# dblalock/sprintz

Hardware: AMD Instinct MI355X
Metric: decompress MB/s (and ratio) uint16 rowmajor 8-col, 1/2/4/8 MI355X vs CPU ref (higher is better)
Workload: dtype u16

## Files before the change

sprintz_amd/csrc/decode_fast.h:

```cpp
#pragma once

#include "decode_kernel.h"
#include "group_ops.h"

namespace sprintz {

typedef uint32_t __attribute__((aligned(1), may_alias)) u32_unaligned;
typedef uint16_t __attribute__((aligned(1), may_alias)) u16_unaligned;
struct __attribute__((aligned(1), packed)) u128_unaligned { uint32_t x, y, z, w; };

typedef __attribute__((address_space(3))) const uint32_t lds_u32;
typedef __attribute__((address_space(3))) const uint8_t lds_u8;

__device__ __forceinline__ uint32_t lds_rd32(uint32_t a)
{
    lds_u32* q = (lds_u32*)(uintptr_t)(a & ~3u);
    return __builtin_amdgcn_alignbyte(q[1], q[0], a);
}
__device__ __forceinline__ uint32_t lds_rd8(uint32_t a) { return *(lds_u8*)(uintptr_t)a; }
__device__ __forceinline__ uint32_t lds_addr(const void* p)
{
    return (uint32_t)(uintptr_t)(__attribute__((address_space(3))) const void*)p;
}

__device__ __forceinline__ uint64_t wave_uniform64(uint64_t x)
{
    return ((uint64_t)(uint32_t)__builtin_amdgcn_readfirstlane((int)(uint32_t)(x >> 32)) << 32) |
           (uint64_t)(uint32_t)__builtin_amdgcn_readfirstlane((int)(uint32_t)x);
}

__device__ __forceinline__ int mad24(int a, int b, int c)
{
    int d;
    asm("v_mad_i32_i24 %0, %1, %2, %3" : "=v"(d) : "v"(a), "v"(b), "v"(c));
    return d;
}
__device__ __forceinline__ int sign_of(int x)
{
    int s;
    asm("v_med3_i32 %0, %1, -1, 1" : "=v"(s) : "v"(x));
    return s;
}

__device__ __forceinline__ int mad_i16_hi(int a, int b, int c)
{
    int d;
    asm("v_mad_i32_i16 %0, %1, %2, %3 op_sel:[1,0,0,0]" : "=v"(d) : "v"(a), "v"(b), "v"(c));
    return d;
}
__device__ __forceinline__ uint32_t add_hi16(uint32_t a, int x)
{
    uint32_t d;
    asm("v_add_u32_sdwa %0, %1, %2 dst_sel:DWORD dst_unused:UNUSED_PAD src0_sel:DWORD src1_sel:WORD_1" : "=v"(d) : "v"(a), "v"(x));
    return d;
}

template <int W, bool FIRE, int DP, int CPL, bool EXACT, int Q = 0, bool CM = false, int DS = 0>
__global__ void __launch_bounds__(kThreads) decode_fast_kernel(DecodeArgs a)
{
    using U = typename Elem<W>::U;
    typedef __attribute__((__vector_size__(4 * sizeof(uint32_t)))) uint32_t v4u;
    constexpr int HB = Elem<W>::HB;
    constexpr int ESZ = W / 8;
    constexpr int LOG2DP = DP == 4 ? 2 : DP == 8 ? 3 : DP == 16 ? 4 : DP == 32 ? 5 : 6;
    constexpr int DCAP = DP * CPL;
    constexpr uint32_t ROW16 = DP * 16;
    constexpr uint32_t UNIT = ROW16 * CPL;
    constexpr bool SPLIT = CPL == 3;
    static_assert(!SPLIT || (W == 8 && DP == 32 && !EXACT && !CM && Q == 0), "the split mapping is built for 8-bit row-major decodes");
    constexpr bool GATHER = Q == kQueryGather;
    static_assert(!GATHER || (!CM && !SPLIT && DS == 0), "gather: row-major destination, plain mappings");
    constexpr int DSZ = DS ? DS : DCAP;
    static_assert(DSZ <= DCAP, "sizing columns");
    constexpr uint32_t HDRMAX = (2 * DSZ * HB + 7) / 8;
    constexpr uint32_t BLKMAX = 8 * DSZ * ESZ;
    constexpr int PIECES = (BLKMAX + ROW16 - 1) / ROW16;
    constexpr uint32_t CG = HDRMAX + 2 * BLKMAX + 4;
    constexpr uint32_t NPEND = (CG + UNIT - 1) / UNIT;
    constexpr uint32_t CSTART = 16 + 8;
    constexpr uint32_t RBU = (2 * (CG + CSTART) + 3 + UNIT - 1) / UNIT + 1;
    constexpr uint32_t RB = RBU * UNIT;
    constexpr uint32_t APRON = (CG + CSTART + 8 + 15) & ~15u;
    static_assert(RB - UNIT >= 2 * (CG + CSTART) + 3, "ring too small for one step of read-ahead");
    static_assert(NPEND <= 3, "pending registers");
    extern __shared__ __attribute__((aligned(16))) uint8_t smem[];

    const int D = EXACT ? DCAP : a.D;
    const uint64_t gtid = (uint64_t)blockIdx.x * kThreads + threadIdx.x;
    const int lane_d = (int)(threadIdx.x & (uint32_t)(DP - 1));
    GatherPiece gp{};
    uint64_t c_sel = (gtid >> LOG2DP) * (uint64_t)a.chunks_per_group;
    if constexpr (GATHER) {
        if (!gather_piece(a, gtid >> LOG2DP, gp)) return;
        if (gp.exists && a.offsets[gp.chunk + 1] > 0xfffffff0ull - 4096u) { if (lane_d == 0) gather_fail(a, gp.range, kErrCorrupt); return; }
        if (!gp.exists) { if (lane_d == 0) gather_fail(a, gp.range, kErrNoRow); return; }
        c_sel = gp.chunk;
    }
    const uint64_t c_first = c_sel;
    if (c_first >= a.nchunks) return;
    const uint64_t c_end = GATHER ? c_first + 1 : (c_first + a.chunks_per_group < a.nchunks) ? c_first + a.chunks_per_group : a.nchunks;

    uint8_t* const ringp = smem + (size_t)(threadIdx.x >> LOG2DP) * a.lds_group_stride;
    const uint32_t ring = lds_addr(ringp);
    uint8_t* const stage = ringp + RB + APRON;

    const uint64_t wave_first = GATHER ? 0 : (((uint64_t)blockIdx.x * kThreads + (threadIdx.x & ~63u)) >> LOG2DP) * (uint64_t)a.chunks_per_group;
    uint64_t wave_base = 0;
    if constexpr (!GATHER) {
        wave_base = a.offsets[wave_first < a.nchunks ? wave_first : 0] & ~(uint64_t)15;
        wave_base = wave_uniform64(wave_base);
    }
    const uint64_t wave_span = ((a.offsets[a.nchunks] - wave_base) + 15) & ~(uint64_t)15;
    const __amdgpu_buffer_rsrc_t rsrc = __builtin_amdgcn_make_buffer_rsrc(
        (void*)(a.comp + wave_base), 0, (uint32_t)(wave_span < 0xffffffffull ? wave_span : 0xffffffffull), 0x00020000);
    const uint32_t rows_per_chunk = CM ? a.chunk_len / (uint32_t)(EXACT ? DCAP : a.D) : 0u;
    const uint64_t out_base = CM ? (wave_first < a.nchunks ? wave_first : 0) * (uint64_t)rows_per_chunk * ESZ
                                 : (wave_first < a.nchunks ? wave_first : 0) * (uint64_t)a.chunk_len * ESZ;
    const uint64_t out_span = CM ? (uint64_t)(EXACT ? DCAP : a.D) * a.col_stride * ESZ - out_base
                            : GATHER ? a.g_nranges * (uint64_t)a.g_rows * (uint64_t)(EXACT ? DCAP : a.D) * ESZ
                                 : a.nchunks * (uint64_t)a.chunk_len * ESZ - out_base;
    const __amdgpu_buffer_rsrc_t orsrc = __builtin_amdgcn_make_buffer_rsrc(
        (void*)((uint8_t*)a.out + wave_uniform64(out_base)), 0,
        (uint32_t)__builtin_amdgcn_readfirstlane((int)(uint32_t)(out_span < 0xfffffff0ull ? out_span : 0xfffffff0ull)), 0x00020000);
    constexpr uint32_t kDropStore = 0xfffffff0u;
#ifndef SPRINTZ_STORE_AUX
#define SPRINTZ_STORE_AUX 2
#endif
#ifndef SPRINTZ_DF_MERGE8
#define SPRINTZ_DF_MERGE8 1
#endif
    constexpr int kStoreAux = SPRINTZ_STORE_AUX;
    const uint32_t lane16 = (uint32_t)lane_d * 16u;
    uint64_t gabs = 0;
    uint32_t gvo = 0;
    uint32_t rp = 0;
    uint32_t rofs = 0;
    uint32_t ahead = 0;
    uint32_t cofs = lane16;

    uint4 pend[3][CPL];
    uint32_t npend = 0;

    auto request = [&](uint4 (&v)[CPL], bool wanted) {
#pragma unroll
        for (int j = 0; j < CPL; j++) {
            const auto t = __builtin_amdgcn_raw_buffer_load_b128(rsrc, wanted ? gvo + j * ROW16 : 0xfffffff0u, 0, 0);
            v[j] = make_uint4(t[0], t[1], t[2], t[3]);
        }
        gvo += wanted ? UNIT : 0u;
    };
    auto commit = [&](const uint4 (&v)[CPL]) {
#pragma unroll
        for (int j = 0; j < CPL; j++) {
            const uint32_t ro = cofs + j * ROW16;
            *(uint4*)(ringp + ro) = v[j];
            if (ro < APRON) *(uint4*)(ringp + RB + ro) = v[j];
        }
        cofs += UNIT;
        if (cofs >= RB) cofs -= RB;
    };
    auto prime = [&](uint64_t off) {
        gabs = off & ~(uint64_t)15;
        gvo = (uint32_t)(gabs - wave_base) + lane16;
        rp = (uint32_t)(off & 15);
        rofs = rp;
        cofs = lane16;
        npend = 0;
        wave_lds_sync();
#pragma unroll
        for (uint32_t u = 0; u < RB / UNIT; u++) {
            uint4 v[CPL];
            request(v, true);
            commit(v);
        }
        ahead = RB - rp;
        wave_lds_sync();
    };

    const uint32_t hdr_bytes = (2u * (uint32_t)D * HB + 7u) >> 3;
    const uint32_t blk_elems = 8u * (uint32_t)D;
    const uint32_t blk_bytes = blk_elems * ESZ;
    const uint32_t row_stride = (uint32_t)D * ESZ;
    const int col0 = lane_d * CPL;
    constexpr bool MERGE8 = SPRINTZ_DF_MERGE8 && W == 8 && (CPL % 2 == 0 || SPLIT) && !CM && Q == 0;
    const bool merge8 = MERGE8 && (EXACT || (D & 1) == 0);
    constexpr int NPAIR = CPL / 2;
    int genk[CPL];
    int colk[CPL];
    uint8_t* stage_k[CPL];
#pragma unroll
    for (int k = 0; k < CPL; k++) {
        genk[k] = SPLIT ? (k < 2 ? 2 * lane_d + k : 2 * DP + lane_d) : col0 + k;
        if (MERGE8 && merge8 && !SPLIT) {
            const int pb = (col0 + (k & ~1)) < D ? col0 + (k & ~1) : ((D - 1) & ~1);
            colk[k] = EXACT ? col0 + k : (pb + (k & 1) < D ? pb + (k & 1) : D - 1);
        } else {
            colk[k] = EXACT ? genk[k] : (genk[k] < D ? genk[k] : D - 1);
        }
        stage_k[k] = stage + colk[k] * ESZ;
    }

    uint32_t pv[CPL];
    int pd[CPL], ctr[CPL];
    bool col_ok[CPL];
#pragma unroll
    for (int k = 0; k < CPL; k++) { pv[k] = 0; pd[k] = 0; ctr[k] = 0; col_ok[k] = EXACT ? true : genk[k] < D; }
    uint32_t out_left = 0;
    bool corrupt = false;
    uint32_t qmax[CPL];
    uint64_t qsum[CPL];
    uint32_t qbs[CPL];
#pragma unroll
    for (int k = 0; k < CPL; k++) { qmax[k] = 0; qsum[k] = 0; qbs[k] = 0; }
    constexpr uint32_t MASK = Elem<W>::MASK;
    uint32_t qmin[CPL];
    uint32_t wi = 0, wleft = 0;
    uint64_t wbase = 0;
    auto q_row = [&](int k) {
        if constexpr (Q != 0) {
            if constexpr (W == 16) {
                asm("v_max_u32_sdwa %0, %1, %2 dst_sel:DWORD dst_unused:UNUSED_PAD src0_sel:DWORD src1_sel:WORD_0"
                    : "=v"(qmax[k]) : "v"(qmax[k]), "v"(pv[k]));
                if constexpr (Q == kQueryWindow)
                    asm("v_min_u32_sdwa %0, %1, %2 dst_sel:DWORD dst_unused:UNUSED_PAD src0_sel:DWORD src1_sel:WORD_0"
                        : "=v"(qmin[k]) : "v"(qmin[k]), "v"(pv[k]));
                asm("v_add_u32_sdwa %0, %1, %2 dst_sel:DWORD dst_unused:UNUSED_PAD src0_sel:DWORD src1_sel:WORD_0"
                    : "=v"(qbs[k]) : "v"(qbs[k]), "v"(pv[k]));
            } else {
                asm("v_max_u32_sdwa %0, %1, %2 dst_sel:DWORD dst_unused:UNUSED_PAD src0_sel:DWORD src1_sel:BYTE_0"
                    : "=v"(qmax[k]) : "v"(qmax[k]), "v"(pv[k]));
                if constexpr (Q == kQueryWindow)
                    asm("v_min_u32_sdwa %0, %1, %2 dst_sel:DWORD dst_unused:UNUSED_PAD src0_sel:DWORD src1_sel:BYTE_0"
                        : "=v"(qmin[k]) : "v"(qmin[k]), "v"(pv[k]));
                asm("v_add_u32_sdwa %0, %1, %2 dst_sel:DWORD dst_unused:UNUSED_PAD src0_sel:DWORD src1_sel:BYTE_0"
                    : "=v"(qbs[k]) : "v"(qbs[k]), "v"(pv[k]));
            }
        }
    };
    auto q_block = [&](int k) {
        if constexpr (Q != 0) { qsum[k] += qbs[k]; qbs[k] = 0; }
    };
    auto win_flush_all = [&]() {
#pragma unroll
        for (int k = 0; k < CPL; k++)
            if (col_ok[k]) win_flush<W>(a, (wbase + wi) * (uint64_t)D + (uint64_t)genk[k], qmin[k], qmax[k], qsum[k]);
        wi++;
        wleft = a.window_rows;
    };
    auto q_window = [&]() {
        if constexpr (Q == kQueryWindow) {
            wleft -= 8;
            if (wleft == 0) win_flush_all();
        }
    };
    uint32_t ovo = 0;
    uint32_t grow = 0;
    uint32_t prow[PIECES];
#pragma unroll
    for (int q = 0; q < PIECES; q++) prow[q] = GATHER ? (lane16 + (uint32_t)q * ROW16) / row_stride : 0u;
    const uint32_t gspan = gp.hi - gp.lo;

    uint4 held[2][PIECES];
    uint32_t held_vo[2][PIECES];
#pragma unroll
    for (int s2 = 0; s2 < 2; s2++)
#pragma unroll
        for (int q = 0; q < PIECES; q++) { held[s2][q] = make_uint4(0, 0, 0, 0); held_vo[s2][q] = kDropStore; }
    uint32_t pk[CPL][4];
    uint4 cheld[2][CPL];
    uint32_t cheld_vo[2][CPL];
    uint32_t cbase[CPL];
#pragma unroll
    for (int k = 0; k < CPL; k++) {
        cbase[k] = CM ? (uint32_t)((uint64_t)genk[k] * a.col_stride * ESZ) : 0u;
#pragma unroll
        for (int s2 = 0; s2 < 2; s2++) { cheld[s2][k] = make_uint4(0, 0, 0, 0); cheld_vo[s2][k] = kDropStore; }
    }
    auto store_col = [&](const uint4& t, uint32_t vo) {
        if constexpr (W == 16) {
            __builtin_amdgcn_raw_buffer_store_b128(__builtin_bit_cast(v4u, t), orsrc, vo, 0, kStoreAux);
        } else {
            typedef __attribute__((__vector_size__(2 * sizeof(uint32_t)))) uint32_t v2u;
            v2u h = {t.x, t.y};
            __builtin_amdgcn_raw_buffer_store_b64(h, orsrc, vo, 0, kStoreAux);
        }
    };
    constexpr bool CMB = CM && CPL == 1;
    constexpr uint32_t PB = W == 16 ? 16u : 8u;
    uint8_t* const cst = stage;
    uint32_t* const cvo = (uint32_t*)(stage + 4u * DCAP * PB);
    uint32_t stepno = 0;
    const uint32_t cs_bytes = CM ? (uint32_t)(a.col_stride * ESZ) : 0u;
    auto cst_at = [&](uint32_t col, uint32_t blk) { return cst + (col * 4u + ((blk + (col >> 2)) & 3u)) * PB; };
    if constexpr (CMB) {
        if (lane_d < 4) cvo[lane_d] = kDropStore;
        wave_lds_sync();
    }
    auto cm_flush = [&](bool real) {
        if constexpr (CMB) {
            wave_lds_sync();
#pragma unroll
            for (int j = 0; j < 4; j++) {
                const uint32_t pid = (uint32_t)j * DP + (uint32_t)lane_d, col = pid >> 2, p = pid & 3u;
                uint4 t = make_uint4(0, 0, 0, 0);
                uint32_t vo = kDropStore;
                if (real && col < (uint32_t)D) {
                    const uint32_t rofs_b = cvo[p];
                    if constexpr (W == 16) t = *(const uint4*)cst_at(col, p);
                    else { const uint2 h = *(const uint2*)cst_at(col, p); t.x = h.x; t.y = h.y; }
                    vo = rofs_b == kDropStore ? kDropStore : col * cs_bytes + rofs_b;
                }
                store_col(t, vo);
            }
            if (real) {
                wave_lds_sync();
                if (lane_d < 4) cvo[lane_d] = kDropStore;
            }
            wave_lds_sync();
        }
    };
    auto pack_row = [&](int k, int i) {
        if constexpr (CM) {
            if constexpr (W == 16) {
                if ((i & 1) == 0) pk[k][i >> 1] = pv[k] & 0xffffu;
                else pk[k][i >> 1] |= pv[k] << 16;
            } else {
                if ((i & 3) == 0) pk[k][i >> 2] = pv[k] & 0xffu;
                else pk[k][i >> 2] |= (pv[k] & 0xffu) << (8 * (i & 3));
            }
        }
    };
    auto stage_out = [&](int slot) {
        if constexpr (query_reduce_only(Q)) return;
        if constexpr (CMB) {
            if (slot >= 0) {
                const uint32_t blk = (stepno & 1u) * 2u + (uint32_t)slot;
                if (col_ok[0]) {
                    if constexpr (W == 16) *(uint4*)cst_at((uint32_t)col0, blk) = make_uint4(pk[0][0], pk[0][1], pk[0][2], pk[0][3]);
                    else *(uint2*)cst_at((uint32_t)col0, blk) = make_uint2(pk[0][0], pk[0][1]);
                }
                if (lane_d == 0) cvo[blk] = ovo;
            } else {
                const uint4 t = W == 16 ? make_uint4(pk[0][0], pk[0][1], pk[0][2], pk[0][3]) : make_uint4(pk[0][0], pk[0][1], 0, 0);
                store_col(t, col_ok[0] ? cbase[0] + ovo : kDropStore);
            }
            ovo += 8u * ESZ;
            return;
        }
        if constexpr (CM) {
#pragma unroll
            for (int k = 0; k < CPL; k++) {
                const uint4 t = W == 16 ? make_uint4(pk[k][0], pk[k][1], pk[k][2], pk[k][3]) : make_uint4(pk[k][0], pk[k][1], 0, 0);
                const uint32_t vo = col_ok[k] ? cbase[k] + ovo : kDropStore;
                if (slot >= 0) { cheld[slot][k] = t; cheld_vo[slot][k] = vo; }
                else store_col(t, vo);
            }
            ovo += 8u * ESZ;
            return;
        }
        wave_lds_sync();
#pragma unroll
        for (int q = 0; q < PIECES; q++) {
            const uint32_t u = lane16 + q * ROW16;
            bool in = u < blk_bytes;
            if constexpr (GATHER) in = in && grow + prow[q] - gp.lo < gspan;
            const uint4 t = *(const uint4*)(stage + (in ? u : 0u));
            if (slot >= 0) {
                held[slot][q] = t;
#ifdef SPRINTZ_ABL_NO_GSTORE
                held_vo[slot][q] = kDropStore;
#elif defined(SPRINTZ_ABL_STORE_INTERLEAVE)
                {
                    const uint32_t g = (threadIdx.x & 63u) >> LOG2DP, gbase = g * a.chunk_len * ESZ;
                    held_vo[slot][q] = in ? ((ovo - gbase) >> 7) * 1024u + g * 128u + u : kDropStore;
                }
#elif defined(SPRINTZ_ABL_STORE_SLOT0_ONLY)
                held_vo[slot][q] = (in && slot == 0) ? ovo + u : kDropStore;
#elif defined(SPRINTZ_ABL_STORE_HALF_LANES)
                held_vo[slot][q] = (in && (lane_d & 1) == 0) ? ovo + u : kDropStore;
#else
                held_vo[slot][q] = in ? ovo + u : kDropStore;
#endif
            } else {
                __builtin_amdgcn_raw_buffer_store_b128(__builtin_bit_cast(v4u, t), orsrc, in ? ovo + u : kDropStore, 0, kStoreAux);
            }
        }
        wave_lds_sync();
        ovo += blk_bytes;
    };
    auto run_blocks = [&](uint32_t len) {
        if constexpr (Q == kQueryWindow && !FIRE) {
            if ((uint64_t)len * blk_elems > out_left) { corrupt = true; return; }
            out_left -= len * blk_elems;
            uint32_t rows = len * 8u;
            while (rows > 0) {
                const uint32_t n = rows < wleft ? rows : wleft;
#pragma unroll
                for (int k = 0; k < CPL; k++) {
                    const uint32_t x = pv[k] & MASK;
                    qmin[k] = x < qmin[k] ? x : qmin[k];
                    qmax[k] = x > qmax[k] ? x : qmax[k];
                    qsum[k] += (uint64_t)x * n;
                }
                rows -= n;
                wleft -= n;
                if (wleft == 0) win_flush_all();
            }
            return;
        }
        if constexpr (GATHER && !FIRE) {
            uint32_t skip = grow + 8u <= gp.lo ? (gp.lo - grow) >> 3 : 0u;
            skip = skip < len ? skip : len;
            if ((uint64_t)skip * blk_elems > out_left) { corrupt = true; return; }
            out_left -= skip * blk_elems;
            ovo += skip * blk_bytes;
            grow += skip * 8u;
            len -= skip;
        }
        for (; len > 0; len--) {
            if constexpr (GATHER) { if (grow >= gp.hi) break; }
            if (out_left < blk_elems) { corrupt = true; break; }
            out_left -= blk_elems;
            auto run_step = [&](int k, int coef) {
                if constexpr (W == 16 && FIRE) {
                    pd[k] = mad_i16_hi(pd[k], coef, 0);
                    pv[k] = add_hi16(pv[k], pd[k]);
                } else {
                    const int delta = FIRE ? __builtin_amdgcn_sbfe(mad24(pd[k], coef, 0), W, W) : 0;
                    pv[k] += (uint32_t)delta;
                    pd[k] = delta;
                }
            };
            auto run_col = [&](int k) {
                int coef = FIRE ? fire_coef<W, false>(ctr[k]) : 0;
                if constexpr (FIRE && W == 16) {
                    if (a.quirk) coef = fire_coef_ref_run16(ctr[k], genk[k]);
                }
#pragma unroll
                for (int i = 0; i < 8; i++) {
                    run_step(k, coef);
                    q_row(k);
                    pack_row(k, i);
#ifndef SPRINTZ_ABL_NO_STAGE
                    if constexpr (!query_reduce_only(Q) && !CM)
                        *(U*)(stage_k[k] + i * row_stride) = (U)pv[k];
#endif
                }
                q_block(k);
            };
            if (MERGE8 && merge8) {
#pragma unroll
                for (int j = 0; j < NPAIR; j++) {
                    const int k = 2 * j;
                    const int coef0 = FIRE ? fire_coef<W, false>(ctr[k]) : 0, coef1 = FIRE ? fire_coef<W, false>(ctr[k + 1]) : 0;
#pragma unroll
                    for (int i = 0; i < 8; i++) {
                        run_step(k, coef0);
                        run_step(k + 1, coef1);
                        *(uint16_t*)(stage_k[k] + i * row_stride) = (uint16_t)__builtin_amdgcn_perm(pv[k + 1], pv[k], 0x0c0c0400u);
                    }
                }
                if constexpr (CPL & 1) run_col(CPL - 1);
            } else {
#pragma unroll
                for (int k = 0; k < CPL; k++) run_col(k);
            }
            q_window();
            if constexpr (GATHER) {
                if (grow + 8u > gp.lo) stage_out(-1); else ovo += blk_bytes;
                grow += 8u;
            } else {
                stage_out(-1);
            }
        }
    };
    auto fetch_rows = [&](int (&e)[CPL][8], uint32_t at, const uint32_t (&off)[CPL], const uint32_t (&nb)[CPL], uint32_t row_bytes) {
        if constexpr (W == 8 && CPL >= 2) {
#pragma unroll
            for (int j = 0; j < NPAIR; j++) {
                const int k = 2 * j;
                uint32_t p = at + (off[k] >> 3);
                const uint32_t sha = off[k] & 7u, shb = off[k + 1] - (off[k] & ~7u);
                const uint32_t w1a = nb[k] != 0 ? 1u : 0u, wma = nb[k] - w1a;
                const uint32_t w1b = nb[k + 1] != 0 ? 1u : 0u, wmb = nb[k + 1] - w1b;
#pragma unroll
                for (int i = 0; i < 8; i++) {
                    const uint32_t w = lds_rd32(p);
                    const uint32_t ea = __builtin_amdgcn_ubfe(w, sha + 1u, wma) ^ (uint32_t)__builtin_amdgcn_sbfe((int)w, sha, w1a);
                    const uint32_t eb = __builtin_amdgcn_ubfe(w, shb + 1u, wmb) ^ (uint32_t)__builtin_amdgcn_sbfe((int)w, shb, w1b);
                    e[k][i] = FIRE ? (int)ea << 8 : (int)ea;
                    e[k + 1][i] = FIRE ? (int)eb << 8 : (int)eb;
                    p += row_bytes;
                }
            }
            if constexpr (CPL % 2 == 0) return;
        }
#pragma unroll
        for (int k = (W == 8 && CPL >= 2) ? 2 * NPAIR : 0; k < CPL; k++) {
            uint32_t p = at + (off[k] >> 3);
            const uint32_t sh = off[k] & 7u;
            const uint32_t w1 = nb[k] != 0 ? 1u : 0u;
            const uint32_t wm = nb[k] - w1;
#pragma unroll
            for (int i = 0; i < 8; i++) {
#ifdef SPRINTZ_ABL_NO_FETCH
                const uint32_t w = p * 2654435761u;
#else
                const uint32_t w = lds_rd32(p);
#endif
                const uint32_t mag = __builtin_amdgcn_ubfe(w, sh + 1u, wm);
                const int sgn = __builtin_amdgcn_sbfe((int)w, sh, w1);
                if constexpr (W == 16) {
                    int x;
                    asm("v_xor_b32_sdwa %0, %1, %2 dst_sel:WORD_1 dst_unused:UNUSED_PAD src0_sel:WORD_0 src1_sel:WORD_0"
                        : "=v"(x) : "v"(mag), "v"(sgn));
                    e[k][i] = x;
                } else if constexpr (FIRE) {
                    e[k][i] = (int)(mag ^ (uint32_t)sgn) << 8;
                } else {
                    e[k][i] = (int)(mag ^ (uint32_t)sgn);
                }
                p += row_bytes;
            }
        }
    };
    auto packed_block = [&](const int (&e)[CPL][8], int slot) {
        if (out_left < blk_elems) { corrupt = true; return; }
        out_left -= blk_elems;
        auto col_step = [&](int k, int i, int coef, int& grad) {
            if constexpr (W == 16 && FIRE) {
                if (i & 1) grad = mad_i16_hi(pd[k], sign_of(e[k][i]), grad);
                pd[k] = mad_i16_hi(pd[k], coef, e[k][i]);
                pv[k] = add_hi16(pv[k], pd[k]);
            } else if constexpr (W == 16) {
                pv[k] = add_hi16(pv[k], e[k][i]);
            } else {
                int delta;
                if constexpr (FIRE) {
                    if (i & 1) grad = mad24(sign_of(e[k][i]), pd[k], grad);
                    delta = __builtin_amdgcn_sbfe(mad24(pd[k], coef, e[k][i]), W, W);
                } else {
                    delta = e[k][i];
                }
                pv[k] += (uint32_t)delta;
                pd[k] = delta;
            }
        };
        auto one_col = [&](int k) {
            int grad = 0;
            const int coef = FIRE ? fire_coef<W, false>(ctr[k]) : 0;
#pragma unroll
            for (int i = 0; i < 8; i++) {
                col_step(k, i, coef, grad);
                q_row(k);
                pack_row(k, i);
#ifndef SPRINTZ_ABL_NO_STAGE
                if constexpr (!query_reduce_only(Q) && !CM)
                    *(U*)(stage_k[k] + i * row_stride) = (U)pv[k];
#else
                asm volatile("" :: "v"(pv[k]));
#endif
            }
            q_block(k);
            if constexpr (FIRE) ctr[k] = wrap_counter<W>(ctr[k] + __builtin_amdgcn_sbfe(grad, 2, W - 2));
        };
        if (MERGE8 && merge8) {
#pragma unroll
            for (int j = 0; j < NPAIR; j++) {
                const int k = 2 * j;
                int grad0 = 0, grad1 = 0;
                const int coef0 = FIRE ? fire_coef<W, false>(ctr[k]) : 0, coef1 = FIRE ? fire_coef<W, false>(ctr[k + 1]) : 0;
#pragma unroll
                for (int i = 0; i < 8; i++) {
                    col_step(k, i, coef0, grad0);
                    col_step(k + 1, i, coef1, grad1);
                    *(uint16_t*)(stage_k[k] + i * row_stride) = (uint16_t)__builtin_amdgcn_perm(pv[k + 1], pv[k], 0x0c0c0400u);
                }
                if constexpr (FIRE) {
                    ctr[k] = wrap_counter<W>(ctr[k] + __builtin_amdgcn_sbfe(grad0, 2, W - 2));
                    ctr[k + 1] = wrap_counter<W>(ctr[k + 1] + __builtin_amdgcn_sbfe(grad1, 2, W - 2));
                }
            }
            if constexpr (CPL & 1) one_col(CPL - 1);
        } else {
#pragma unroll
            for (int k = 0; k < CPL; k++) one_col(k);
        }
        q_window();
        stage_out(slot);
        if constexpr (GATHER) grow += 8u;
    };
    auto run_length = [&](uint32_t at, uint32_t& nbytes) -> uint32_t {
        const uint32_t b0 = lds_rd8(at);
        uint32_t len = b0 & 0x7fu;
        nbytes = 1;
        if (b0 & 0x80u) { len |= lds_rd8(at + 1) << 7; nbytes = 2; }
        return len;
    };

    bool need_prime = true;
    for (uint64_t chunk = c_first; chunk < c_end; chunk++) {
    const uint64_t off_c = a.offsets[chunk];
    {
        const uint64_t off = off_c;
        const uint64_t gap = off - (gabs + rp);
        if (need_prime || gap > 16 || rp > (1u << 30)) {
            prime(off);
        } else {
            rp += (uint32_t)gap;
            rofs += (uint32_t)gap;
            if (rofs >= RB) rofs -= RB;
            ahead -= (uint32_t)gap;
        }
        need_prime = false;
    }
    uint32_t groups_left, remaining;
    {
        const uint32_t w0 = lds_rd32(ring + rofs), w1 = lds_rd32(ring + rofs + 4);
        uint32_t hbytes = 8, nd_hdr = w1 >> 16;
        groups_left = w0;
        remaining = w1 & 0xffffu;
        if (a.norle) {
            const uint32_t len = w0 <= a.chunk_len ? w0 : 0u;
            nd_hdr = w0 <= a.chunk_len ? (a.norle == 2 ? w1 >> 16 : w1 & 0xffffu) : 0xffffffffu;
            hbytes = a.norle == 2 ? 8u : 6u;
            groups_left = len < 128u ? 0u : len / (16u * (uint32_t)D);
            remaining = len - groups_left * 16u * (uint32_t)D;
        }
        rp += hbytes;
        rofs += hbytes;
        if (rofs >= RB) rofs -= RB;
        ahead -= hbytes;
#pragma unroll
        for (int k = 0; k < CPL; k++) { pv[k] = 0; pd[k] = 0; ctr[k] = 0; qmax[k] = 0; qsum[k] = 0; }
        if constexpr (Q == kQueryWindow) {
#pragma unroll
            for (int k = 0; k < CPL; k++) qmin[k] = MASK;
            wi = 0;
            wleft = a.window_rows;
            wbase = chunk * (uint64_t)a.win_count;
        }
        out_left = a.chunk_len;
        ovo = CM ? (uint32_t)((chunk - wave_first) * (uint64_t)rows_per_chunk * ESZ)
          : GATHER ? (uint32_t)(uint64_t)(gp.obase * ESZ)
                 : (uint32_t)((chunk - wave_first) * (uint64_t)a.chunk_len * ESZ);
        corrupt = (int)nd_hdr != D;
        const uint64_t stream_len = a.offsets[chunk + 1] - off_c;
        if ((uint64_t)groups_left * (hdr_bytes + (a.norle ? 0u : 2u)) > stream_len || groups_left > a.chunk_len / blk_elems + 2u) corrupt = true;
        if (corrupt) groups_left = 0;
    }

    while (groups_left > 0 && !corrupt) {
        if constexpr (GATHER) { if (grow >= gp.hi) break; }
        groups_left--;
        {
            const uint32_t room = RB - ahead;
            {
            npend = 0;
#pragma unroll
            for (uint32_t k = 0; k < NPEND; k++) {
                const bool wanted = room >= (k + 1) * UNIT;
                request(pend[k], wanted);
                npend += wanted ? 1u : 0u;
            }
            ahead += npend * UNIT;
            }
        }

        const uint32_t r = ring + rofs;
        uint32_t nb_both[CPL], lane_both = 0;
        uint32_t hw0 = 0, hw1 = 0;
#pragma unroll
        for (int k = 0; k < CPL; k++) {
            const uint32_t hbit0 = (uint32_t)colk[k] * HB, hbit1 = (uint32_t)(D + colk[k]) * HB;
            uint32_t s0 = hbit0 & 7u, s1 = hbit1 & 7u;
            if (k & 1) {
                const uint32_t b0 = (uint32_t)colk[k - 1] * HB, b1 = (uint32_t)(D + colk[k - 1]) * HB;
                s0 = hbit0 - (b0 & ~7u);
                s1 = hbit1 - (b1 & ~7u);
            } else {
                hw0 = lds_rd32(r + (hbit0 >> 3));
                hw1 = lds_rd32(r + (hbit1 >> 3));
            }
            uint32_t f0 = __builtin_amdgcn_ubfe(hw0, s0, HB);
            uint32_t f1 = __builtin_amdgcn_ubfe(hw1, s1, HB);
            f0 += (f0 == (uint32_t)(W - 1));
            f1 += (f1 == (uint32_t)(W - 1));
            nb_both[k] = f0 | (f1 << 16);
            lane_both += col_ok[k] ? nb_both[k] : 0u;
        }
        uint32_t tot_both;
        uint32_t excl_both, excl_single = 0;
        if constexpr (SPLIT) {
            uint32_t tot_pairs, tot_singles;
            excl_both = group_scan<DP>(nb_both[0] + nb_both[1], lane_d, tot_pairs);
            excl_single = tot_pairs + group_scan<DP>(col_ok[2] ? nb_both[2] : 0u, lane_d, tot_singles);
            tot_both = tot_pairs + tot_singles;
        } else {
            excl_both = group_scan<DP>(lane_both, lane_d, tot_both);
        }
        const uint32_t tot0 = tot_both & 0xffffu, tot1 = tot_both >> 16;
        uint32_t off0[CPL], off1[CPL], nb0[CPL], nb1[CPL];
#pragma unroll
        for (int k = 0; k < CPL; k++) {
            uint32_t o_both = col_ok[k] ? (SPLIT && k == 2 ? excl_single : excl_both) : tot_both - nb_both[k];
            if constexpr (MERGE8 && !EXACT && !SPLIT) {
                if ((k & 1) == 0 && !col_ok[k] && colk[k] != colk[k + 1]) o_both -= nb_both[k + 1];
            }
            off0[k] = o_both & 0xffffu;
            off1[k] = o_both >> 16;
            nb0[k] = nb_both[k] & 0xffffu;
            nb1[k] = nb_both[k] >> 16;
            excl_both += nb_both[k];
        }

        const uint32_t at0 = r + hdr_bytes;
        uint32_t len0 = 0, len1 = 0, bytes0, bytes1;
        const uint32_t rb0 = (tot0 + 7u) >> 3, rb1 = (tot1 + 7u) >> 3;
        if (tot0 == 0) { if (a.norle) { len0 = 1; bytes0 = 0; } else len0 = run_length(at0, bytes0); } else bytes0 = rb0 * 8u;
        const uint32_t at1 = at0 + bytes0;
        if (tot1 == 0) { if (a.norle) { len1 = 1; bytes1 = 0; } else len1 = run_length(at1, bytes1); } else bytes1 = rb1 * 8u;
        const uint32_t used = hdr_bytes + bytes0 + bytes1;
        int z0[CPL][8], z1[CPL][8];
        if (tot0 != 0) fetch_rows(z0, at0, off0, nb0, rb0);
        if (tot1 != 0) fetch_rows(z1, at1, off1, nb1, rb1);

        if (tot0 == 0) run_blocks(len0); else packed_block(z0, 0);
        if (!corrupt && !(GATHER && grow >= gp.hi)) { if (tot1 == 0) run_blocks(len1); else packed_block(z1, 1); }

        rp += used;
        rofs += used;
        if (rofs >= RB) rofs -= RB;
        ahead -= used;

        if constexpr (!query_reduce_only(Q) && CMB) {
            cm_flush((stepno & 1u) != 0);
            stepno++;
        } else if constexpr (!query_reduce_only(Q) && CM) {
#pragma unroll
            for (int s2 = 0; s2 < 2; s2++)
#pragma unroll
                for (int k = 0; k < CPL; k++) store_col(cheld[s2][k], cheld_vo[s2][k]);
        } else if constexpr (!query_reduce_only(Q)) {
#pragma unroll
            for (int s2 = 0; s2 < 2; s2++)
#pragma unroll
                for (int q = 0; q < PIECES; q++)
                    __builtin_amdgcn_raw_buffer_store_b128(__builtin_bit_cast(v4u, held[s2][q]), orsrc, held_vo[s2][q], 0, kStoreAux);
        }
#pragma unroll
        for (uint32_t k = 0; k < NPEND; k++)
            if (k < npend) commit(pend[k]);
        wave_lds_sync();
    }

    if constexpr (CMB) {
        if (stepno & 1u) cm_flush(true);
        stepno = 0;
    }
    const uint32_t out_elems = a.chunk_len - out_left;
    if constexpr (GATHER) {
        if (corrupt) { if (lane_d == 0) gather_fail(a, gp.range, kErrCorrupt); return; }
        if (grow >= gp.hi) return;
        if (remaining > out_left || (uint64_t)gp.hi * (uint32_t)D > (uint64_t)out_elems + remaining) {
            if (lane_d == 0) gather_fail(a, gp.range, remaining > out_left ? kErrCorrupt : kErrNoRow);
            return;
        }
        if (gabs + rp + (uint64_t)remaining * ESZ > a.offsets[chunk + 1]) { if (lane_d == 0) gather_fail(a, gp.range, kErrCorrupt); return; }
        const uint8_t* t = a.comp + gabs + rp;
        const uint32_t e_lo = gp.lo * (uint32_t)D > out_elems ? gp.lo * (uint32_t)D - out_elems : 0u;
        const uint32_t e_hi = gp.hi * (uint32_t)D - out_elems;
        U* const d = (U*)a.out + (gp.obase + (int64_t)out_elems);
        for (uint32_t e = e_lo + (uint32_t)lane_d; e < e_hi; e += DP)
            d[e] = ESZ == 1 ? (U)t[e] : (U)*(const u16_unaligned*)(t + 2 * e);
        return;
    }
    if (!corrupt && remaining > out_left) corrupt = true;
    if constexpr (Q == kQueryWindow) {
        if (!corrupt) {
            const uint8_t* t = a.comp + gabs + rp;
#pragma unroll
            for (int k = 0; k < CPL; k++) {
                if (!col_ok[k]) continue;
                uint32_t w = wi, left = wleft;
                for (uint32_t e = (uint32_t)genk[k]; e < remaining; e += (uint32_t)D) {
                    if (left == 0) {
                        win_flush<W>(a, (wbase + w) * (uint64_t)D + (uint64_t)genk[k], qmin[k], qmax[k], qsum[k]);
                        w++;
                        left = a.window_rows;
                    }
                    left--;
                    const uint32_t x = ESZ == 1 ? (uint32_t)t[e] : (uint32_t)*(const u16_unaligned*)(t + 2 * e);
                    qmin[k] = x < qmin[k] ? x : qmin[k];
                    qmax[k] = x > qmax[k] ? x : qmax[k];
                    qsum[k] += x;
                }
                for (; w < a.win_count; w++) win_flush<W>(a, (wbase + w) * (uint64_t)D + (uint64_t)genk[k], qmin[k], qmax[k], qsum[k]);
            }
        }
    } else if constexpr (Q != 0) {
        if (!corrupt) {
            const uint8_t* t = a.comp + gabs + rp;
#pragma unroll
            for (int k = 0; k < CPL; k++) {
                if (!col_ok[k]) continue;
                for (uint32_t e = (uint32_t)genk[k]; e < remaining; e += (uint32_t)D) {
                    const uint32_t x = ESZ == 1 ? (uint32_t)t[e] : (uint32_t)*(const u16_unaligned*)(t + 2 * e);
                    qmax[k] = x > qmax[k] ? x : qmax[k];
                    qsum[k] += x;
                }
                if (a.qres) a.qres[chunk * (uint64_t)D + (uint64_t)genk[k]] = a.qop == 1 ? (uint64_t)qmax[k] : qsum[k];
            }
        }
    }
    if (!corrupt && remaining > 0 && !query_reduce_only(Q) && CM) {
        const uint8_t* t = a.comp + gabs + rp;
        U* const c0 = (U*)((uint8_t*)a.out + out_base + ovo);
        for (uint32_t e = (uint32_t)lane_d; e < remaining; e += DP) {
            const uint32_t x = ESZ == 1 ? (uint32_t)t[e] : (uint32_t)*(const u16_unaligned*)(t + 2 * e);
            c0[(uint64_t)(e % (uint32_t)D) * a.col_stride + e / (uint32_t)D] = (U)x;
        }
    } else if (!corrupt && remaining > 0 && !query_reduce_only(Q)) {
        const uint8_t* t = a.comp + gabs + rp;
        uint8_t* d = (uint8_t*)a.out + out_base + ovo;
        copy_verbatim(t, d, remaining * ESZ, (uint32_t)lane_d, (uint32_t)DP);
    }
    if (corrupt || remaining > 0) need_prime = true;
    if (lane_d == 0 && a.rets) a.rets[chunk] = corrupt ? kErrCorrupt : (int64_t)out_elems + remaining;
    }
}

constexpr uint32_t decode_fast_lds_bytes(int W, int DP, int CPL, int D, bool colmajor_burst = false, int DS = 0)
{
    const uint32_t unit = DP * 16 * CPL;
    const uint32_t hb = W == 8 ? 3 : 4;
    const uint32_t dcap = DS ? DS : DP * CPL;
    const uint32_t hdrmax = (2 * dcap * hb + 7) / 8, blkmax = 8 * dcap * (W / 8);
    const uint32_t cg = hdrmax + 2 * blkmax + 4;
    const uint32_t rb = ((2 * (cg + 24) + 3 + unit - 1) / unit + 1) * unit;
    const uint32_t apron = (cg + 24 + 8 + 15) & ~15u;
    const uint32_t stage = colmajor_burst ? 4u * blkmax + 16 : ((8u * D * (W / 8) + 15) & ~15u) + 16;
    return rb + apron + stage;
}

}
```

Measured before the change: 3.354 million.

## Move ring read-ahead to step end and batch prime loads for single-column decodes

For configurations with one column per lane (such as u16 with CPL=1), global read-ahead requests now go out after the step's consumption. They are committed before the next step rather than at its top, which gives loads a full step to land. A wave ballot skips request issue when no lane needs room. The prime phase now issues all ring-unit loads before committing any, so the loads overlap. Chunk offsets are also loaded up front and carried across iterations instead of being reread. This adds register pressure from holding RBU units at once and the reordering could change LDS/commit timing.

```diff
diff --git a/sprintz_amd/csrc/decode_fast.h b/sprintz_amd/csrc/decode_fast.h
--- a/sprintz_amd/csrc/decode_fast.h
+++ b/sprintz_amd/csrc/decode_fast.h
@@ -54,6 +54,16 @@
     asm("v_add_u32_sdwa %0, %1, %2 dst_sel:DWORD dst_unused:UNUSED_PAD src0_sel:DWORD src1_sel:WORD_1" : "=v"(d) : "v"(a), "v"(x));
     return d;
 }
+
+#ifndef SPRINTZ_DF_REQ_AT_TOP
+#define SPRINTZ_DF_REQ_AT_TOP 0
+#endif
+#ifndef SPRINTZ_DF_REQ_UNGUARDED
+#define SPRINTZ_DF_REQ_UNGUARDED 0
+#endif
+#ifndef SPRINTZ_DF_SERIAL_START
+#define SPRINTZ_DF_SERIAL_START 0
+#endif
 
 template <int W, bool FIRE, int DP, int CPL, bool EXACT, int Q = 0, bool CM = false, int DS = 0>
 __global__ void __launch_bounds__(kThreads) decode_fast_kernel(DecodeArgs a)
@@ -69,6 +79,8 @@
     constexpr bool SPLIT = CPL == 3;
     static_assert(!SPLIT || (W == 8 && DP == 32 && !EXACT && !CM && Q == 0), "the split mapping is built for 8-bit row-major decodes");
     constexpr bool GATHER = Q == kQueryGather;
+    constexpr bool REQ_TOP = SPRINTZ_DF_REQ_AT_TOP || CPL > 1 || GATHER || (W == 8 && (CM || Q == kQueryReduceOnly || Q == kQueryWindow));
+    constexpr bool BATCH_START = !REQ_TOP && !SPRINTZ_DF_SERIAL_START;
     static_assert(!GATHER || (!CM && !SPLIT && DS == 0), "gather: row-major destination, plain mappings");
     constexpr int DSZ = DS ? DS : DCAP;
     static_assert(DSZ <= DCAP, "sizing columns");
@@ -99,6 +111,13 @@
     const uint64_t c_first = c_sel;
     if (c_first >= a.nchunks) return;
     const uint64_t c_end = GATHER ? c_first + 1 : (c_first + a.chunks_per_group < a.nchunks) ? c_first + a.chunks_per_group : a.nchunks;
+    uint64_t off_first = 0, off_second = 0;
+    uint64_t off_end = a.offsets[a.nchunks];
+    if constexpr (BATCH_START) {
+        off_first = a.offsets[c_first];
+        off_second = a.offsets[c_first + 1];
+        asm volatile("" : "+s"(off_end));
+    }
 
     uint8_t* const ringp = smem + (size_t)(threadIdx.x >> LOG2DP) * a.lds_group_stride;
     const uint32_t ring = lds_addr(ringp);
@@ -107,10 +126,11 @@
     const uint64_t wave_first = GATHER ? 0 : (((uint64_t)blockIdx.x * kThreads + (threadIdx.x & ~63u)) >> LOG2DP) * (uint64_t)a.chunks_per_group;
     uint64_t wave_base = 0;
     if constexpr (!GATHER) {
-        wave_base = a.offsets[wave_first < a.nchunks ? wave_first : 0] & ~(uint64_t)15;
+        if constexpr (BATCH_START) wave_base = off_first & ~(uint64_t)15;
+        else wave_base = a.offsets[wave_first < a.nchunks ? wave_first : 0] & ~(uint64_t)15;
         wave_base = wave_uniform64(wave_base);
     }
-    const uint64_t wave_span = ((a.offsets[a.nchunks] - wave_base) + 15) & ~(uint64_t)15;
+    const uint64_t wave_span = ((off_end - wave_base) + 15) & ~(uint64_t)15;
     const __amdgpu_buffer_rsrc_t rsrc = __builtin_amdgcn_make_buffer_rsrc(
         (void*)(a.comp + wave_base), 0, (uint32_t)(wave_span < 0xffffffffull ? wave_span : 0xffffffffull), 0x00020000);
     const uint32_t rows_per_chunk = CM ? a.chunk_len / (uint32_t)(EXACT ? DCAP : a.D) : 0u;
@@ -167,14 +187,39 @@
         cofs = lane16;
         npend = 0;
         wave_lds_sync();
-#pragma unroll
-        for (uint32_t u = 0; u < RB / UNIT; u++) {
-            uint4 v[CPL];
-            request(v, true);
-            commit(v);
+        if constexpr (BATCH_START) {
+            uint4 v[RBU][CPL];
+#pragma unroll
+            for (uint32_t u = 0; u < RBU; u++) request(v[u], true);
+#pragma unroll
+            for (uint32_t u = 0; u < RBU; u++) commit(v[u]);
+        } else {
+#pragma unroll
+            for (uint32_t u = 0; u < RBU; u++) {
+                uint4 v[CPL];
+                request(v, true);
+                commit(v);
+            }
         }
         ahead = RB - rp;
         wave_lds_sync();
+    };
+
+    auto request_units = [&]() {
+        const uint32_t room = RB - ahead;
+        npend = 0;
+#pragma unroll
+        for (uint32_t k = 0; k < NPEND; k++) {
+            const bool wanted = room >= (k + 1) * UNIT;
+            if (REQ_TOP || SPRINTZ_DF_REQ_UNGUARDED || __builtin_amdgcn_ballot_w64(wanted) != 0) request(pend[k], wanted);
+            npend += wanted ? 1u : 0u;
+        }
+        ahead += npend * UNIT;
+    };
+    auto commit_pending = [&]() {
+#pragma unroll
+        for (uint32_t k = 0; k < NPEND; k++)
+            if (k < npend) commit(pend[k]);
     };
 
     const uint32_t hdr_bytes = (2u * (uint32_t)D * HB + 7u) >> 3;
@@ -599,8 +644,9 @@
     };
 
     bool need_prime = true;
+    uint64_t off_c = off_first, off_next = off_second;
     for (uint64_t chunk = c_first; chunk < c_end; chunk++) {
-    const uint64_t off_c = a.offsets[chunk];
+    if constexpr (!BATCH_START) off_c = a.offsets[chunk];
     {
         const uint64_t off = off_c;
         const uint64_t gap = off - (gabs + rp);
@@ -645,7 +691,8 @@
           : GATHER ? (uint32_t)(uint64_t)(gp.obase * ESZ)
                  : (uint32_t)((chunk - wave_first) * (uint64_t)a.chunk_len * ESZ);
         corrupt = (int)nd_hdr != D;
-        const uint64_t stream_len = a.offsets[chunk + 1] - off_c;
+        if constexpr (!BATCH_START) off_next = a.offsets[chunk + 1];
+        const uint64_t stream_len = off_next - off_c;
         if ((uint64_t)groups_left * (hdr_bytes + (a.norle ? 0u : 2u)) > stream_len || groups_left > a.chunk_len / blk_elems + 2u) corrupt = true;
         if (corrupt) groups_left = 0;
     }
@@ -653,19 +700,7 @@
     while (groups_left > 0 && !corrupt) {
         if constexpr (GATHER) { if (grow >= gp.hi) break; }
         groups_left--;
-        {
-            const uint32_t room = RB - ahead;
-            {
-            npend = 0;
-#pragma unroll
-            for (uint32_t k = 0; k < NPEND; k++) {
-                const bool wanted = room >= (k + 1) * UNIT;
-                request(pend[k], wanted);
-                npend += wanted ? 1u : 0u;
-            }
-            ahead += npend * UNIT;
-            }
-        }
+        if constexpr (REQ_TOP) request_units();
 
         const uint32_t r = ring + rofs;
         uint32_t nb_both[CPL], lane_both = 0;
@@ -733,6 +768,10 @@
         if (rofs >= RB) rofs -= RB;
         ahead -= used;
 
+        if constexpr (!REQ_TOP) {
+            commit_pending();
+            request_units();
+        }
         if constexpr (!query_reduce_only(Q) && CMB) {
             cm_flush((stepno & 1u) != 0);
             stepno++;
@@ -748,9 +787,7 @@
                 for (int q = 0; q < PIECES; q++)
                     __builtin_amdgcn_raw_buffer_store_b128(__builtin_bit_cast(v4u, held[s2][q]), orsrc, held_vo[s2][q], 0, kStoreAux);
         }
-#pragma unroll
-        for (uint32_t k = 0; k < NPEND; k++)
-            if (k < npend) commit(pend[k]);
+        if constexpr (REQ_TOP) commit_pending();
         wave_lds_sync();
     }
 
@@ -827,6 +864,9 @@
     }
     if (corrupt || remaining > 0) need_prime = true;
     if (lane_d == 0 && a.rets) a.rets[chunk] = corrupt ? kErrCorrupt : (int64_t)out_elems + remaining;
+    if constexpr (BATCH_START) {
+        if (chunk + 1 < c_end) { off_c = a.offsets[chunk + 1]; off_next = a.offsets[chunk + 2]; }
+    }
     }
 }
 
```

Result: faster. 3.407 million, median of 6 (+1.6%).
